# zyrlia1018/CMD-GEN

Measured on AMD Instinct MI355X. Metric: denoising steps/sec, higher is better.
Workload: dtype f32

## Files before the change

### cmdgen_amd/csrc/cmdgen_api.hip

```cpp
#include "cmdgen_dev.h"
#include "../../include/cmdgen_hip.h"

#include <cmath>
#include <cstdarg>
#include <cstdio>
#include <cstring>
#include <cstdlib>
#include <map>
#include <string>
#include <vector>

void cmdgen_launch_eval(const EvalLaunch& a, const float* xh_phar, const float* xh_pocket,
                        const float* t_arr, const float4* coef, ChainState* chain, float* eps_phar,
                        float* eps_pocket, hipStream_t s, hipEvent_t* ev);
void cmdgen_launch_nan_fix(const EvalLaunch& a, float* eps_phar, hipStream_t s);
void cmdgen_readout_allow_lds(size_t bytes);
void cmdgen_launch_edges(const EvalLaunch& a, const float* xh_phar, const float* xh_pocket, hipStream_t s);
void cmdgen_build_pocket_cache(const EvalLaunch& a, const float* xh_phar, const float* xh_pocket, const float* t01,
                               float* c, float* P0, float* Q0, float* dh, float* dP, float* dQ, hipStream_t s);
void cmdgen_launch_edge_msg_only(const EvalLaunch& a, int layer, hipStream_t s);
void cmdgen_launch_chain_init(const Layout& lay, const Dims& d, const ChainBuf& c, const float* px,
                              const float* poh, hipStream_t s);
void cmdgen_launch_step_count(const Layout& lay, const Dims& d, const ChainBuf& c, const Work& w,
                              const float* eps, hipStream_t s);
// ... 588 lines not shown
    const bool sp256 = h->dims.H == 256 && h->gemm_split;
    if (!sp256) { if (a.edge_mt == 128) a.edge_mt = 64; if (a.coord_mt == 128) a.coord_mt = 64; }
    if (h->dims.sin && h->dims.H == 512) { if (a.edge_mt > 32) a.edge_mt = 32; if (a.coord_mt > 32) a.coord_mt = 32; }
    a.edge_fullk = (sp256 && opt_of(h, "edge_fullk", 1) != 0) ? 1 : 0;
    a.e128_wgs = (int)opt_of(h, "e128_wgs_per_cu", 2);
    a.e128_fused = h->e128_fused;
    {
        const int he = (int)opt_of(h, "half_engine", 1);
        a.half_engine = he == 2 || (he == 1 && h->dims.cutoff2 >= 0.f) ? 1 : 0;
    }
    a.write_embed = opt_of(h, "write_embed", 1) != 0 ? 1 : 0;
    {
        int on = 0;
        if (sp256 && h->n_cus > 0 && h->have_layout) {
            const int ncu = h->n_cus, t64 = (h->lay.N + 63) / 64, t32 = (h->lay.N + 31) / 32;
            const float cost64 = (float)((t64 + ncu - 1) / ncu);
            const int full = t32 / (2 * ncu), rem = t32 - full * 2 * ncu;
            float cost32 = 1.12f * full + (rem == 0 ? 0.f : rem <= ncu ? 0.62f : 1.12f);
            if (a.half_engine) cost32 = 1.9f * full + (rem == 0 ? 0.f : rem <= ncu ? 1.22f : 1.9f);
            on = cost64 < cost32 && !(a.half_engine && h->node_mt == 16);
            if (a.half_engine && h->node_mt != 16) on = 32;
            if (on == 32 && t32 > ncu && t64 <= ncu) on = 8;
            else if (on == 32 && t64 > ncu) on = 2;
            if (opt_set(h, "node64")) { const int64_t v = opt_of(h, "node64", 0); on = v == 32 ? 32 : v == 8 ? 8 : v == 2 ? 2 : v != 0; }
        }
        a.node64 = on;
        a.dead_skip = (h->dims.joint || h->dims.S != 1) ? 0 : (int)opt_of(h, "dead_skip", 2);
        if (!on && !a.dead_skip) a.w.need_qc = nullptr;
        a.w.hop_levels = a.dead_skip >= 2 ? h->dims.L : 1;
        if (!a.dead_skip) a.w.ehop = nullptr;
    }
    a.split16 = (a.split && h->dims.H >= 128 && opt_of(h, "node16_split", 1) != 0) ? 1 : 0;
    a.node16w = opt_of(h, "node16w", 1) != 0 ? 1 : 0;
    {
        a.embed_mt = (int)opt_of(h, "embed_mt", (((double)h->lay.Nl / 16.0 <= 2.0 * h->n_cus && !h->dims.joint) ? 16 : a.node_mt));
        if (a.embed_mt != 16 && a.embed_mt != 32 && a.embed_mt != 64) a.embed_mt = a.node_mt;
    }
    if (a.split && a.node_mt == 64 && !opt_set(h, "node_mt")) a.node_mt = 32;
    return a;
}

static const char* const kOptionKeys[] = {
    "node_mt", "edge_mt", "coord_mt", "embed_mt", "edge_wgs_per_cu", "coord_wgs_per_cu", "e128_wgs_per_cu", "e128_fused", "half_engine", "edge_fullk", "node64", "node16_split", "node16w",
    "dead_skip", "write_embed", "graph_steps",
    "wgrad_split", "wgrad_tile", "wgrad_split_wgs128", "wgrad_split_wgs64", "wgrad_wgs", "dgrad_mt", "dgrad_tail", "wgrad_stream", "train_half", "wgrad_silu", "train_node16", "wgrad_k128"};

static void drop_graphs(cmdgen_handle* h) {
    hipSetDevice(h->device);
    if (h->own_stream) hipStreamSynchronize(h->own_stream);
    if (h->have_layout) hipStreamSynchronize(h->last_stream);
    drop_chain_graphs(h);
}
static void refresh_tune(cmdgen_handle* h) {
    TrainTune t;
    t.wgrad_split = (int)opt_of(h, "wgrad_split", t.wgrad_split); t.wgrad_tile = (int)opt_of(h, "wgrad_tile", t.wgrad_tile);
    t.wgrad_split_wgs128 = (int)opt_of(h, "wgrad_split_wgs128", t.wgrad_split_wgs128); t.wgrad_split_wgs64 = (int)opt_of(h, "wgrad_split_wgs64", t.wgrad_split_wgs64);
    t.wgrad_wgs = (int)opt_of(h, "wgrad_wgs", t.wgrad_wgs); t.dgrad_mt = (int)opt_of(h, "dgrad_mt", t.dgrad_mt); t.dgrad_tail = (int)opt_of(h, "dgrad_tail", t.dgrad_tail);
    t.wgrad_stream = (int)opt_of(h, "wgrad_stream", t.wgrad_stream); t.wgrad_k128 = (int)opt_of(h, "wgrad_k128", t.wgrad_k128);
    h->tune = t;
}

extern "C" int cmdgen_set_option(cmdgen_handle* h, const char* key, int64_t value, int32_t unset) {
    if (!h || !key) return fail(h, CMDGEN_EINVAL, "null argument");
    bool known = false;
    for (const char* k : kOptionKeys) known = known || strcmp(k, key) == 0;
    if (!known) return fail(h, CMDGEN_EINVAL, "unknown option '%s'", key);
    drop_graphs(h);
    if (unset) h->opts.erase(key); else h->opts[key] = value;
    refresh_tune(h);
    if (h->have_layout) pick_tiles(h);
    return CMDGEN_OK;
}

extern "C" int cmdgen_get_option(cmdgen_handle* h, const char* key, int64_t* value, int32_t* is_set) {
    if (!h || !key) return fail(h, CMDGEN_EINVAL, "null argument");
    bool known = false;
// ... 63 lines not shown
    TMP(w.ed0, float, need); TMP(w.totals, int, 4); TMP(w.counters, unsigned long long, 8); TMP(w.nan_flag, int, 4);
#undef TMP
    if (rc) { free_pool(pool); return rc; }
    w.erow = row_dev; w.ecol = col_dev;
    hipMemcpy(d_np, cnt.data(), B * sizeof(int), hipMemcpyHostToDevice);
    hipMemcpy(d_base, base.data(), B * sizeof(int), hipMemcpyHostToDevice);
    L.B = B; L.Nl = 0; L.Np = (int)N; L.N = (int)N; L.Nm = 0; L.max_n = max_n;
    L.num_phar = d_zero; L.num_pocket = d_np; L.phar_base = d_zero; L.pocket_base = d_base;
    EvalLaunch a{}; a.lay = L; a.w = w; a.d = d;
    cmdgen_launch_edges(a, x , x, s);
    hipError_t e = hipStreamSynchronize(s);
    int tot[2] = {0, 0};
    if (e == hipSuccess) e = hipMemcpy(tot, w.totals, sizeof tot, hipMemcpyDeviceToHost);
    free_pool(pool);
    if (e != hipSuccess) return fail(h, CMDGEN_EHIP, "radius graph failed: %s", hipGetErrorString(e));
    *n_edges = tot[0];
    return CMDGEN_OK;
}

extern "C" int cmdgen_get_edges(cmdgen_handle* h, int32_t* row, int32_t* col, int64_t cap, int64_t* n_edges, cmdgen_stream stream) {
    int rc = check_ready(h); if (rc) return rc;
    hipSetDevice(h->device);
    hipStream_t s = (hipStream_t)stream;
    HIPCHK(h, hipStreamSynchronize(s));
    int tot[2];
    HIPCHK(h, hipMemcpy(tot, h->work.totals, sizeof tot, hipMemcpyDeviceToHost));
    if (n_edges) *n_edges = tot[0];
    const int64_t n = tot[0] < cap ? tot[0] : cap;
    if (n > 0 && row) HIPCHK(h, hipMemcpy(row, h->work.erow, n * sizeof(int), hipMemcpyDeviceToHost));
    if (n > 0 && col) HIPCHK(h, hipMemcpy(col, h->work.ecol, n * sizeof(int), hipMemcpyDeviceToHost));
    return CMDGEN_OK;
}

extern "C" int cmdgen_debug_read(cmdgen_handle* h, const char* what, float* host, size_t n, cmdgen_stream stream) {
    int rc = check_ready(h); if (rc) return rc;
    hipSetDevice(h->device);
    HIPCHK(h, hipStreamSynchronize((hipStream_t)stream));
    const void* src = nullptr; size_t have = 0;
    const std::string k = what ? what : "";
    const Dims& d = h->dims;
    if (k == "h") { src = h->work.h; have = (size_t)h->lay.N * d.H; }
    else if (k == "agg") { src = h->work.agg; have = (size_t)h->lay.N * d.H; }
    else if (k == "P") { src = h->work.P; have = (size_t)h->lay.N * d.H; }
    else if (k == "Q") { src = h->work.Q; have = (size_t)h->lay.N * d.H; }
    else if (k == "x0") { src = h->work.X0; have = (size_t)h->lay.Nm * 4; }
    else if (k == "xl") { src = h->work.XL; have = (size_t)d.L * h->lay.Nm * 4; }
    else if (k == "acc") { src = h->work.ACC; have = (size_t)d.L * h->lay.Nm * 4; }
    else return fail(h, CMDGEN_EINVAL, "unknown debug buffer '%s'", k.c_str());
    if (n > have) n = have;
    HIPCHK(h, hipMemcpy(host, src, n * sizeof(float), hipMemcpyDeviceToHost));
    return CMDGEN_OK;
}

static inline float softplus_f(float x) { return x > 20.f ? x : log1pf(expf(x)); }
static inline float logsigmoid_f(float x) { return -softplus_f(-x); }
static inline float sigmoid_h(float x) { return 1.0f / (1.0f + expf(-x)); }

static void build_step_table(const std::vector<float>& gamma, int T, int K, std::vector<float>& coef) {
    coef.assign((size_t)(K + 1) * 4, 0.f);
    for (int i = 0; i < K; ++i) {
        const int s = K - 1 - i;
        const float s_arr = (float)s / (float)K, t_arr = (float)(s + 1) / (float)K;
        const float g_s = gamma[(size_t)lrintf(s_arr * (float)T)], g_t = gamma[(size_t)lrintf(t_arr * (float)T)];
        const float sigma2_ts = -expm1f(softplus_f(g_s) - softplus_f(g_t));
        const float alpha_ts = expf(0.5f * (logsigmoid_f(-g_t) - logsigmoid_f(-g_s)));
        const float sigma_ts = sqrtf(sigma2_ts);
        const float sigma_s = sqrtf(sigmoid_h(g_s)), sigma_t = sqrtf(sigmoid_h(g_t));
        coef[i * 4 + 0] = alpha_ts;
        coef[i * 4 + 1] = sigma2_ts / alpha_ts / sigma_t;
        coef[i * 4 + 2] = sigma_ts * sigma_s / sigma_t;
        coef[i * 4 + 3] = t_arr;
    }
    const float g0 = gamma[0];
    coef[K * 4 + 0] = sqrtf(sigmoid_h(g0));
    coef[K * 4 + 1] = sqrtf(sigmoid_h(-g0));
    coef[K * 4 + 2] = expf(0.5f * g0);
    coef[K * 4 + 3] = 0.f;
}

extern "C" int cmdgen_set_step_table(cmdgen_handle* h, int32_t K, const float* coef_host) {
// ... 588 lines not shown
    if (which == 1) {
        if (h256 && a.split && sampler && a.node64 && lw.W3.ws) return a.half_engine && lw.W3.wh ? 3 : 6;
        if (h256 && a.node_mt == 16 && a.split16 && a.node16w && sampler && lw.W3.ws16) return a.half_engine && lw.W3.wh16 ? 3 : 6;
        if ((a.split && a.node_mt >= 32) || (a.split16 && a.node_mt == 16)) return 6;
        return 1;
    }
    const int mt = which == 0 ? a.edge_mt : a.coord_mt;
    const WPack& W = which == 0 ? lw.W2 : lw.W7;
    if (mt == 128 && h256 && a.split && sampler && W.ws) return a.half_engine && W.wh ? 3 : 6;
    if (a.edge_fullk && sampler && a.split && h256 && mt == 32) return a.half_engine && W.wh ? 3 : 6;
    if (a.split && mt >= 32) return 6;
    return 1;
}

extern "C" int cmdgen_query(cmdgen_handle* h, const char* key, int64_t* value) {
    if (!h || !key || !value) return CMDGEN_EINVAL;
    if (!h->have_layout) return fail(h, CMDGEN_ESTATE, "no batch layout (cmdgen_set_layout)");
    const std::string k = key;
    const EvalLaunch a = make_launch(h);
    if (k == "node_mt") *value = a.node_mt;
    else if (k == "edge_mt") *value = a.edge_mt;
    else if (k == "e128_fused") *value = a.e128_fused;
    else if (k == "coord_mt") *value = a.coord_mt;
    else if (k == "edge_grid") *value = a.edge_grid;
    else if (k == "coord_grid") *value = a.coord_grid;
    else if (k == "gemm_split") *value = a.split;
    else if (k == "half_engine") *value = a.split ? a.half_engine : 0;
    else if (k == "msg_mfmas_per_product") *value = mfmas_per_product(a, 0);
    else if (k == "node_mfmas_per_product") *value = mfmas_per_product(a, 1);
    else if (k == "coord_mfmas_per_product") *value = mfmas_per_product(a, 2);
    else if (k == "node16_split") *value = a.split16;
    else if (k == "node64") *value = a.node64;
    else if (k == "node16w") *value = a.node16w;
    else if (k == "edge_fullk") *value = a.edge_fullk;
    else if (k == "dead_skip") *value = a.dead_skip;
    else if (k == "eval_gen") *value = h->eval_gen;
    else if (k == "train_half_ran") *value = h->train_fwd_half;
    else if (k == "train_range_event") *value = h->h_norm && !h->norm_pending ? (int64_t)h->h_norm[1] : 0;
    else if (k == "train_edges") *value = h->train_E;
    else if (k == "train_coord_edges") *value = h->train_Ec;
    else return fail(h, CMDGEN_EINVAL, "unknown query '%s'", key);
    return CMDGEN_OK;
}

extern "C" int cmdgen_time_evaluation(cmdgen_handle* h, const float* xh_phar, const float* xh_pocket, const float* t,
                                      float* eps_phar, int32_t graph_len, int32_t replays, float* mean_ms, cmdgen_stream stream) {
    int rc = check_ready(h); if (rc) return rc;
    if (!xh_phar || !xh_pocket || !t || !eps_phar || !mean_ms || graph_len < 1 || replays < 1) return fail(h, CMDGEN_EINVAL, "bad arguments");
    if (h->dims.joint) return fail(h, CMDGEN_ESTATE, "cmdgen_time_evaluation supports the conditional model only");
    hipStream_t caller = (hipStream_t)stream, s = caller;
    if (caller == nullptr) {
        rc = own_stream(h); if (rc) return rc;
        HIPCHK(h, hipDeviceSynchronize());
        s = h->own_stream;
    }
    rc = begin_work(h, s); if (rc) return rc;
    EvalLaunch a = make_launch(h);
    ++h->eval_gen;
    hipGraph_t g = nullptr; hipGraphExec_t ge = nullptr;
    hipEvent_t e0 = nullptr, e1 = nullptr;
    hipError_t err = hipStreamBeginCapture(s, hipStreamCaptureModeThreadLocal);
    if (err != hipSuccess) return fail(h, CMDGEN_EHIP, "hipStreamBeginCapture: %s", hipGetErrorString(err));
    for (int i = 0; i < graph_len; ++i) {
        cmdgen_launch_eval(a, xh_phar, xh_pocket, t, nullptr, nullptr, eps_phar, nullptr, s, nullptr);
        cmdgen_launch_nan_fix(a, eps_phar, s);
    }
// ... 92 lines not shown
```

### cmdgen_amd/csrc/cmdgen_dev.h

```cpp
#pragma once
#include <hip/hip_runtime.h>
#include <stdint.h>
#include <vector>
#include "cmdgen_split.h"

typedef float f32x16 __attribute__((ext_vector_type(16)));

#define CMDGEN_MAX_LAYERS 16
#define CMDGEN_MAX_SMALL 64


struct WPack {
    const float4* w32;
    const float4* w16;
    const void*   ws;
    const void*   ws16;
    const void*   wh;
    const void*   wh16;
    float         wh_scale;
    float         wh_inv;
    const float*  wh_dev;
};

struct LayerW {
// ... 161 lines not shown
    int slot;
};

struct TrainTune {
    int wgrad_split = -1;
    int wgrad_tile = 0;
    int wgrad_k128 = 131072;
    int wgrad_split_wgs128 = 384, wgrad_split_wgs64 = 512;
    int wgrad_wgs = 768;
    int dgrad_mt = 0;
    int dgrad_tail = 1;
    unsigned long long* dbg = nullptr;
    int wgrad_stream = 1;
};

struct EvalLaunch {
    Layout lay; Work w; Dims d; SmallW sw;
    const LayerW* layers;
    int edge_grid, coord_grid;
    int node_mt, edge_mt, coord_mt;
    int embed_mt = 16;
    std::vector<hipEvent_t>* prof_events;
    mutable hipEvent_t pe_start = nullptr, pe_stop = nullptr;
    int ablate;
    int stop_block = -1, stop_stage = 0;
    const TrainSave* save = nullptr;
    PocketCache pcache{};
    int skip_count = 0;
    int split = 0;
    int split16 = 0;
    int n_cus = 256;
    int edge_fullk = 0;
    int node16w = 1;
    int node64 = 0;
    int dead_skip = 0;
    mutable int unit = -1;
    mutable int skip_pc = 0;
    mutable int frag_launches = 0;
    mutable int live_thr = 0;
    int save_half = 0;
    int save_half16 = 0;
    int save_split = 0;
    int write_embed = 1;
    int e128_wgs = 2;
    int e128_fused = 3;
    int half_engine = 1;
};
inline int unit_of(const EvalLaunch& a, int l) { return a.unit >= 0 ? a.unit : l; }
inline int unit_has_next(const EvalLaunch& a, int l) { return unit_of(a, l) + 1 < a.d.L * a.d.S ? 1 : 0; }
inline int node_flags(const EvalLaunch& a, int l) { return unit_has_next(a, l) | (a.live_thr << 1) | (a.skip_pc << 30); }


__device__ __forceinline__ float silu_f(float v) {
    return v * __builtin_amdgcn_rcpf(1.0f + __builtin_amdgcn_exp2f(-1.4426950408889634f * v));
}
__device__ __forceinline__ float sigmoid_f(float v) {
    return __builtin_amdgcn_rcpf(1.0f + __builtin_amdgcn_exp2f(-1.4426950408889634f * v));
}
__device__ __forceinline__ float dist2(const float4& a, const float4& b) {
    const float dx = a.x - b.x, dy = a.y - b.y, dz = a.z - b.z;
    return __fmaf_rn(dz, dz, __fmaf_rn(dy, dy, dx * dx));
}

typedef float f32x4v __attribute__((ext_vector_type(4)));

template <int MT> struct TileAcc;
// ... 249 lines not shown
```

### cmdgen_amd/csrc/cmdgen_node16w_body.h

```cpp
#ifndef NW_RD_HALF
#define NW_RD_HALF 8
#endif
constexpr int NW_H = 256, NW_MT = 16, NW_LD = NW_H + 4 , NW_RD = NW_NPL == 2 ? NW_RD_HALF : 4;
constexpr int NPL = NW_NPL;
constexpr unsigned KBS = 64u * NPL;
#if NW_NPL == 3
typedef sbf16x8 wfrag;
#define NW_MFMA(A, B, C) __builtin_amdgcn_mfma_f32_16x16x32_bf16(A, B, C, 0, 0, 0)
#else
typedef sf16x8 wfrag;
#define NW_MFMA(A, B, C) __builtin_amdgcn_mfma_f32_16x16x32_f16(A, B, C, 0, 0, 0)
#endif
__device__ __forceinline__ const void* nw_pack(const WPack& W) { return NPL == 3 ? W.ws16 : W.wh16; }
__device__ __forceinline__ float nw_scale(const WPack& W) { return NPL == 3 ? 1.0f : W.wh_scale; }
__device__ __forceinline__ float nw_inv(const WPack& W) { return NPL == 3 ? 1.0f : W.wh_inv; }

__device__ __forceinline__ void nw_barrier() { asm volatile("s_waitcnt lgkmcnt(0)\n\ts_barrier" ::: "memory"); }

struct NwFrag { const wfrag* p; unsigned ns; };
__device__ __forceinline__ NwFrag nw_frag(const void* Ws16, int kb32_total, int kb0, int nt0) {
    const int lane = threadIdx.x & 63;
    NwFrag f;
    f.p = reinterpret_cast<const wfrag*>(Ws16) + ((size_t)nt0 * kb32_total + kb0) * KBS + lane;
    f.ns = (unsigned)kb32_total * KBS;
    return f;
}
struct NwRing { wfrag b[NW_RD][2][NPL]; };
__device__ __forceinline__ void nw_load_set(const wfrag* q, unsigned ns, wfrag (&dst)[2][NPL]) {
#pragma unroll
    for (int n = 0; n < 2; ++n)
#pragma unroll
        for (int s = 0; s < NPL; ++s) dst[n][s] = q[n * ns + s * 64];
}
__device__ __forceinline__ void nw_prefetch(const NwFrag& f, NwRing& c) {
#pragma unroll
    for (int i = 0; i < NW_RD - 1; ++i) nw_load_set(f.p + i * KBS, f.ns, c.b[i]);
}

#if NW_NPL == 3
__device__ __forceinline__ void nw_split8(const float4& lo, const float4& hi, wfrag (&p)[NPL]) { split8(lo, hi, p[0], p[1], p[2]); }
#else
__device__ __forceinline__ void nw_split8(const float4& lo, const float4& hi, wfrag (&p)[NPL]) {
    {
        uint32_t a[4], b[4];
        split2_pair(lo.x, lo.y, a[0], b[0]); split2_pair(lo.z, lo.w, a[1], b[1]);
        split2_pair(hi.x, hi.y, a[2], b[2]); split2_pair(hi.z, hi.w, a[3], b[3]);
        typedef uint32_t u4 __attribute__((ext_vector_type(4)));
        const u4 va = {a[0], a[1], a[2], a[3]}, vb = {b[0], b[1], b[2], b[3]};
        p[0] = __builtin_bit_cast(wfrag, va); p[1] = __builtin_bit_cast(wfrag, vb);
    }
}
#endif

template <int KB32>
__device__ __forceinline__ void nw_gemm(const float* ldsA, const NwFrag cur, const NwFrag next, sf32x4 (&acc)[2], NwRing& ring) {
    static_assert(KB32 % NW_RD == 0 && (NW_RD == 4 || NW_RD == 8), "K must be a multiple of the ring's k-range");
    const int lane = threadIdx.x & 63;
    const float* ap = ldsA + (lane & 15) * NW_LD + (lane >> 4) * 4;
    float4 raw[2][2];
    wfrag a[2][NPL];
#define NW_LOADA(SET, PTR) { raw[SET][0] = *reinterpret_cast<const float4*>(PTR); raw[SET][1] = *reinterpret_cast<const float4*>((PTR) + 16); }
#define NW_SPLIT(DST, SET) nw_split8(raw[SET][0], raw[SET][1], a[DST]);
#define NW_MF(AS, AI, BS, BI) _Pragma("unroll") for (int n = 0; n < 2; ++n) acc[n] = NW_MFMA(a[AS][AI], ring.b[BS][n][BI], acc[n]);
#if NW_NPL == 3
#define NW_MFMAS(AS, BS) NW_MF(AS, 2, BS, 0) NW_MF(AS, 1, BS, 1) NW_MF(AS, 0, BS, 2) NW_MF(AS, 1, BS, 0) NW_MF(AS, 0, BS, 1) NW_MF(AS, 0, BS, 0)
#define NW_INTERLEAVE()                                                                                                     \
    _Pragma("unroll") for (int i = 0; i < 12; ++i) {                                                                        \
        __builtin_amdgcn_sched_group_barrier(0x008, 1, 0);                                                                  \
        __builtin_amdgcn_sched_group_barrier(0x002, 4, 0); }
// ... 33 lines not shown
}

template <class F>
__device__ __forceinline__ void nw_foreach(const sf32x4 (&acc)[2], int wave, F f) {
    const int lane = threadIdx.x & 63;
#pragma unroll
    for (int n = 0; n < 2; ++n)
#pragma unroll
        for (int r = 0; r < 4; ++r) f(4 * (lane >> 4) + r, wave * 32 + n * 16 + (lane & 15), n, acc[n][r]);
}
struct NwCol { float v[2]; };
__device__ __forceinline__ NwCol nw_col(const float* __restrict__ vec, int wave) {
    const int lane = threadIdx.x & 63;
    NwCol c;
#pragma unroll
    for (int n = 0; n < 2; ++n) c.v[n] = vec[wave * 32 + n * 16 + (lane & 15)];
    return c;
}
__device__ __forceinline__ void nw_zero(sf32x4 (&acc)[2]) {
#pragma unroll
    for (int n = 0; n < 2; ++n)
#pragma unroll
        for (int r = 0; r < 4; ++r) acc[n][r] = 0.0f;
}
__device__ __forceinline__ void nw_store(const sf32x4 (&acc)[2], int wave, float* __restrict__ out, int row0, int nvalid, const NwCol* bias, float inv) {
    nw_foreach(acc, wave, [&](int row, int col, int n, float v) {
        if (row < nvalid) out[(size_t)(row0 + row) * NW_H + col] = __fmaf_rn(v, inv, bias ? bias->v[n] : 0.f);
    });
}
__device__ __forceinline__ float nw_silu_scaled(float a, float c1, float sc) {
    const float u = __builtin_amdgcn_exp2f(a * c1);
    return a * __builtin_amdgcn_rcpf(__fmaf_rn(u, sc, sc));
}
template <bool SAVE>
__global__ __launch_bounds__(512) void k_node16w(Layout lay, Work w, Dims d, LayerW lw, LayerW lw_next, int layer, int has_next_arg, TrainSave sv) {
    __shared__ __attribute__((aligned(16))) float buf0[NW_MT * NW_LD];
    __shared__ __attribute__((aligned(16))) float buf1[NW_MT * NW_LD];
    const int has_next = has_next_arg & 1;
    const bool skip_pc = ((has_next_arg >> 30) & 1) != 0;
    const int tid = threadIdx.x, wave = tid >> 6;
    const int row0 = (int)blockIdx.x * NW_MT, nvalid = min(NW_MT, lay.N - row0);
    const bool want_pc = row0 < lay.Nm;
    constexpr int KB = NW_H / 32;
    const NwFrag f3a = nw_frag(nw_pack(lw.W3), 2 * KB, 0, 2 * wave), f3b = nw_frag(nw_pack(lw.W3), 2 * KB, KB, 2 * wave);
    const NwFrag f4 = nw_frag(nw_pack(lw.W4), KB, 0, 2 * wave);
    const NwFrag fcp = nw_frag(nw_pack(lw.Wpq_c), KB, 0, 2 * wave), fcq = nw_frag(nw_pack(lw.Wpq_c), KB, 0, NW_H / 16 + 2 * wave);
    const NwFrag fnp = nw_frag(nw_pack(lw_next.Wpq_e), KB, 0, 2 * wave), fnq = nw_frag(nw_pack(lw_next.Wpq_e), KB, 0, NW_H / 16 + 2 * wave);
    NwRing ring;
    nw_prefetch(f3a, ring);
    NwCol b3v = nw_col(lw.b3, wave);
    const NwCol b4v = nw_col(lw.b4, wave), b6v = nw_col(lw.b6, wave), b1nv = nw_col(lw_next.b1, wave);
    float sc3 = nw_scale(lw.W3), inv3 = nw_inv(lw.W3), inv4 = nw_inv(lw.W4), invc = nw_inv(lw.Wpq_c), invn = nw_inv(lw_next.Wpq_e);
    if constexpr (SAVE) { sc3 = lw.W3.wh_dev[0]; inv3 = lw.W3.wh_dev[1]; inv4 = lw.W4.wh_dev[1]; invc = lw.Wpq_c.wh_dev[1]; invn = lw_next.Wpq_e.wh_dev[1]; }
    const float c13 = -1.4426950408889634f * inv3;
    b3v.v[0] *= sc3; b3v.v[1] *= sc3;
    if (layer >= 1 && tid < NW_MT) {
        const int n = row0 + tid;
        if (tid < nvalid && n < lay.Nm) {
            const float4 p = (layer == 1) ? w.X0[n] : w.XL[(size_t)(layer - 1) * lay.Nm + n];
            const float4 a = w.ACC[(size_t)(layer - 1) * lay.Nm + n];
            const float dv = agg_div(w, d, n);
            w.XL[(size_t)layer * lay.Nm + n] = make_float4(p.x + a.x / dv, p.y + a.y / dv, p.z + a.z / dv, 0.f);
        }
    }
    {
        float4 hv[2], av[2];
#pragma unroll
        for (int j = 0; j < 2; ++j) {
            const int idx = tid + 512 * j, r = idx >> 6, c4 = idx & 63;
            hv[j] = make_float4(0.f, 0.f, 0.f, 0.f); av[j] = hv[j];
            if (r < nvalid) {
                hv[j] = reinterpret_cast<const float4*>(w.h + (size_t)(row0 + r) * NW_H)[c4];
                av[j] = reinterpret_cast<const float4*>(w.agg + (size_t)(row0 + r) * NW_H)[c4];
            }
        }
#pragma unroll
        for (int j = 0; j < 2; ++j) {
            const int idx = tid + 512 * j, r = idx >> 6, c4 = idx & 63;
            if (r < nvalid) reinterpret_cast<float4*>(w.agg + (size_t)(row0 + r) * NW_H)[c4] = make_float4(0.f, 0.f, 0.f, 0.f);
            float4 v = av[j];
            const float dv = r < nvalid ? agg_div(w, d, row0 + r) : 1.0f;
            v.x /= dv; v.y /= dv; v.z /= dv; v.w /= dv;
            if (SAVE && r < nvalid) reinterpret_cast<float4*>(sv.aggn + ((size_t)sv.slot * lay.N + row0 + r) * NW_H)[c4] = v;
            *reinterpret_cast<float4*>(buf0 + r * NW_LD + 4 * c4) = hv[j];
            *reinterpret_cast<float4*>(buf1 + r * NW_LD + 4 * c4) = v;
        }
    }
#if CMDGEN_STAMPS == 7
    unsigned long long nst_[8] = {0, 0, 0, 0, 0, 0, 0, 0}, nst_t = __builtin_amdgcn_s_memtime();
    const unsigned long long nst_begin = nst_t;
#define NSTAMP(i) do { const unsigned long long n_ = __builtin_amdgcn_s_memtime(); nst_[i] += n_ - nst_t; nst_t = n_; } while (0)
#else
#define NSTAMP(i) do {} while (0)
#endif
    nw_barrier();
    NSTAMP(0);
    sf32x4 acc[2];
    nw_zero(acc);
    nw_gemm<KB>(buf0, f3a, f3b, acc, ring);
    nw_gemm<KB>(buf1, f3b, f4, acc, ring);
    NSTAMP(1);
    nw_barrier();
    nw_foreach(acc, wave, [&](int row, int col, int n, float v) {
        const float t = nw_silu_scaled(v + b3v.v[n], c13, sc3);
        buf1[row * NW_LD + col] = t;
        if (SAVE && row < nvalid) {
            const size_t o = ((size_t)sv.slot * lay.N + row0 + row) * NW_H + col;
            sv.pre3[o] = (v + b3v.v[n]) * inv3; sv.nact[o] = t;
        }
    });
    nw_barrier();
    NSTAMP(2);
    nw_zero(acc);
    const NwFrag fc = skip_pc ? fnp : want_pc ? fcp : fcq;
    nw_gemm<KB>(buf1, f4, fc, acc, ring);
    if constexpr (NPL == 2) {
        const int row = tid >> 5, c8 = (tid & 31) * 8;
        const float m = fmaxf(absmax4(*reinterpret_cast<const float4*>(buf1 + row * NW_LD + c8)), absmax4(*reinterpret_cast<const float4*>(buf1 + row * NW_LD + c8 + 4)));
        const unsigned long long big = __ballot(m >= HALF_LOW_TAU);
        const int r0 = 2 * wave;
        if ((tid & 63) == 0) half_low_count(w.counters, (r0 < nvalid && (unsigned)big == 0u ? 1u : 0u) + (r0 + 1 < nvalid && (big >> 32) == 0ull ? 1u : 0u));
    }
    NSTAMP(3);
    nw_barrier();
    nw_foreach(acc, wave, [&](int row, int col, int n, float v) {
        float hn = 0.f;
        if (row < nvalid) {
            hn = buf0[row * NW_LD + col] + __fmaf_rn(v, inv4, b4v.v[n]);
            w.h[(size_t)(row0 + row) * NW_H + col] = hn;
            if (SAVE) sv.h[((size_t)(sv.slot + 1) * lay.N + row0 + row) * NW_H + col] = hn;
        }
        buf1[row * NW_LD + col] = hn;
    });
    nw_barrier();
    NSTAMP(4);
    if (want_pc && !skip_pc) {
        nw_zero(acc);
        nw_gemm<KB>(buf1, fcp, fcq, acc, ring);
        nw_store(acc, wave, w.Pc, row0, nvalid, &b6v, invc);
    }
    if (!skip_pc) {
        nw_zero(acc);
        nw_gemm<KB>(buf1, fcq, has_next ? fnp : fcq, acc, ring);
        nw_store(acc, wave, w.Qc, row0, nvalid, nullptr, invc);
    }
    NSTAMP(5);
    if (has_next) {
        nw_zero(acc);
        nw_gemm<KB>(buf1, fnp, fnq, acc, ring);
        nw_store(acc, wave, w.P, row0, nvalid, &b1nv, invn);
        nw_zero(acc);
        nw_gemm<KB>(buf1, fnq, fnq, acc, ring);
        nw_store(acc, wave, w.Q, row0, nvalid, nullptr, invn);
    }
    NSTAMP(6);
#if CMDGEN_STAMPS == 7
    if ((tid & 63) == 0 && wave < 4) {
        for (int i = 0; i < 7; ++i) atomicAdd(&w.dbg[wave * 8 + i], nst_[i]);
        atomicAdd(&w.dbg[32 + wave], __builtin_amdgcn_s_memtime() - nst_begin);
        atomicAdd(&w.dbg[40], 1ull);
    }
#endif
#undef NSTAMP
}
```

### cmdgen_amd/csrc/cmdgen_train.hip

```cpp
#include "cmdgen_host.h"
#include <functional>

void cmdgen_launch_edges(const EvalLaunch& a, const float* xh_phar, const float* xh_pocket, hipStream_t s);
void cmdgen_launch_eval(const EvalLaunch& a, const float* xh_phar, const float* xh_pocket, const float* t_arr, const float4* coef,
                        ChainState* chain, float* eps_phar, float* eps_pocket, hipStream_t s, hipEvent_t* ev);
void cmdgen_launch_nan_fix(const EvalLaunch& a, float* eps_phar, hipStream_t s);
void cmdgen_launch_save_positions(const EvalLaunch& a, float4* X, hipStream_t s);
struct RepackFrag { int src_off, ld, out, in, row_split, col_shift; float* dst32; float* dst16; };
struct RepackMisc { int src_off, ld, rows, cols; float* dst; };
void tr_repack(const float* theta, const void* frag_tab, int n_frag, int max_frag4, const void* misc_tab, int n_misc, int max_misc,
               hipStream_t s);
void cmdgen_sgemm(bool ta, bool tb, int M, int N, int K, const float* A, int lda, const float* B, int ldb, float* C,
                  int ldc, const float* bias, float alpha, bool accumulate, int split_k, hipStream_t s,
                  int epi = 0, float* aux = nullptr, int ldaux = 0, bool bf16 = false);
struct WgradBatch {
    const float* dy[8]; const float* x[8]; float* dw[8]; float* db[8];
    int M[8], N[8], lddy[8], ldx[8], ldw[8];
    int n;
    int xs[8] = {0, 0, 0, 0, 0, 0, 0, 0};
};
void cmdgen_wgrad_group(const WgradBatch& g, int K, bool bf16, hipStream_t s, bool split3 = false, bool force3 = false);
struct RepackSplitT { int src_off, ld; void* dst; int transpose; };
void tr_repack_split_t(const float* theta, const void* tab, int n, hipStream_t s);
struct RepackHalf { int src_off, ld; void* dst; float* sc; int transpose; };
// ... 351 lines not shown
                   bool bias, bool accumulate, hipStream_t s, float* act = nullptr) {
    cmdgen_sgemm(false, true, M, r.out, in, x, ldx, theta + r.w + col0, r.in, y, ldy, (bias && r.has_bias) ? theta + r.b : nullptr,
                 1.0f, accumulate, 1, s, act ? 1 : 0, act, ldy, use_bf16(in));
}
static void linear_dgrad(const float* theta, const PRef& r, int col0, int in, int M, const float* dy, int lddy, float* dx,
                         int lddx, bool accumulate, hipStream_t s, const float* pre = nullptr) {
    cmdgen_sgemm(false, false, M, in, r.out, dy, lddy, theta + r.w + col0, r.in, dx, lddx, nullptr, 1.0f, accumulate, 1, s,
                 pre ? 2 : 0, const_cast<float*>(pre), lddx, use_bf16(r.out));
}
static void linear_wgrad(float* grad, const PRef& r, int col0, int in, int M, const float* dy, int lddy, const float* x,
                         int ldx, hipStream_t s) {
    cmdgen_sgemm(true, false, r.out, in, M, dy, lddy, x, ldx, grad + r.w + col0, r.in, nullptr, 1.0f, true, 0, s, 0, nullptr, 0,
                 g_bf16 && r.out >= 64 && in >= 64);
}

extern "C" int cmdgen_param_count(cmdgen_handle* h, int64_t* n) {
    if (!h || !n) return CMDGEN_EINVAL;
    ParamTable t; build_table(h->dims, t);
    *n = (int64_t)t.total;
    return CMDGEN_OK;
}

extern "C" int cmdgen_param_offset(cmdgen_handle* h, const char* name, int64_t* offset, int64_t* count) {
    if (!h || !name) return CMDGEN_EINVAL;
    ParamTable t; build_table(h->dims, t);
    const std::string k = name;
    for (const PRef* r : t.order) {
        if (k == r->name + ".weight") { if (offset) *offset = (int64_t)r->w; if (count) *count = (int64_t)r->out * r->in; return CMDGEN_OK; }
        if (r->has_bias && k == r->name + ".bias") { if (offset) *offset = (int64_t)r->b; if (count) *count = r->out; return CMDGEN_OK; }
    }
    return fail(h, CMDGEN_EINVAL, "no trainable tensor '%s'", name);
}

extern "C" int cmdgen_train_forward(cmdgen_handle* h, const float* theta, const float* xh_phar, const float* xh_pocket,
                                    const float* t_arr, float* eps_phar, float* eps_pocket, cmdgen_stream stream) {
    if (!h) return CMDGEN_EINVAL;
    if (!h->have_layout) return fail(h, CMDGEN_ESTATE, "no batch layout (cmdgen_set_layout)");
    if (!theta || !xh_phar || !xh_pocket || !t_arr || !eps_phar) return fail(h, CMDGEN_EINVAL, "null device pointer");
    if (h->dims.joint && !eps_pocket) return fail(h, CMDGEN_EINVAL, "the joint model's loss needs eps_pocket");
    hipSetDevice(h->device);
    int rc = ensure_state(h); if (rc) return rc;
    TrainState* t = h->train;
    hipStream_t s = (hipStream_t)stream;
    h->last_stream = s;
    const Dims& d = h->dims;
    const int N = h->lay.N, Nl = h->lay.Nl, Np = h->lay.Np, H = d.H, L = d.L, P = d.P, R = d.R, J = d.J;
    const int ldp = 3 + P, ldq = 3 + R, ld1 = 2 * H + 2;
    EvalLaunch a = make_launch(h);
    ++h->eval_gen;
    a.dead_skip = 0; a.w.need_qc = nullptr; a.w.ehop = nullptr; a.w.hop_levels = 1;
    cmdgen_launch_edges(a, xh_phar, xh_pocket, s);
    if (!t->h_tot) {
        HIPCHK(h, hipHostMalloc((void**)&t->h_tot, 4 * sizeof(int), hipHostMallocDefault));
        HIPCHK(h, hipEventCreateWithFlags(&t->tot_ev, hipEventDisableTiming));
    }
    HIPCHK(h, hipMemcpyAsync(t->h_tot, h->work.totals, 2 * sizeof(int), hipMemcpyDeviceToHost, s));
    HIPCHK(h, hipEventRecord(t->tot_ev, s));
    const bool fwd_half = h->gemm_split && H == 256 && a.half_engine && a.edge_fullk && t->n_half > 0 && opt_of(h, "train_half", 1) != 0;
    if (fwd_half && opt_of(h, "train_node16", 1) != 0) a.node_mt = 16;
    const bool node_half = fwd_half && a.node_mt == 16 && t->n_half16 > 0 && opt_of(h, "train_half", 1) != 2;
    const bool frag_partial = fwd_half && node_half;
    tr_repack(theta, t->frag_tab, frag_partial ? 1 : t->n_frag, t->max_frag4, t->misc_tab, t->n_misc, t->max_misc, s);
    if (h->gemm_split || t->bf16) tr_repack_split_t(theta, t->split_tab, t->n_split, s);
    t->split_packs_valid = (h->gemm_split || t->bf16) && t->n_split > 0;
    if (fwd_half) tr_repack_half(theta, t->half_tab, t->n_half_fwd, t->n_half_fwd, s);
    if (node_half) tr_repack_half16(theta, t->half16_tab, t->n_half16, t->max_half16, s);
// ... 583 lines not shown
```

### cmdgen_amd/csrc/kernels_node16w.hip

```cpp
#include "cmdgen_dev.h"
#include "cmdgen_split.h"
#include <hip/hip_ext.h>

#define NW_NPL 2
namespace nw_half {
#include "cmdgen_node16w_body.h"
}
#undef NW_NPL
#undef NW_MFMA
#define NW_NPL 3
namespace nw_bf3 {
#include "cmdgen_node16w_body.h"
}
#undef NW_NPL
#undef NW_MFMA

bool cmdgen_launch_node16w(const EvalLaunch& a, int l, hipStream_t s) {
    const LayerW& lw = a.layers[unit_of(a, l)];
    const LayerW& ln = a.layers[unit_has_next(a, l) ? unit_of(a, l) + 1 : unit_of(a, l)];
    const int nt = (a.lay.N + 15) / 16;
    if (a.save) {
        if (a.d.H != 256 || a.node_mt != 16 || !a.save_half16 || !lw.W3.wh16 || !lw.W3.wh_dev) return false;
        TrainSave sv = *a.save; sv.slot = unit_of(a, l);
        hipLaunchKernelGGL(nw_half::k_node16w<true>, dim3(nt), dim3(512), 0, s, a.lay, a.w, a.d, lw, ln, l, node_flags(a, l), sv);
        return true;
    }
    if (a.d.H != 256 || a.node_mt != 16 || !a.split16 || !a.node16w || !lw.W3.ws16) return false;
    if (a.half_engine && lw.W3.wh16) {
        if (a.pe_start) hipExtLaunchKernelGGL(nw_half::k_node16w<false>, dim3(nt), dim3(512), 0, s, a.pe_start, a.pe_stop, 0, a.lay, a.w, a.d, lw, ln, l, node_flags(a, l), TrainSave{});
        else hipLaunchKernelGGL(nw_half::k_node16w<false>, dim3(nt), dim3(512), 0, s, a.lay, a.w, a.d, lw, ln, l, node_flags(a, l), TrainSave{});
    } else {
        if (a.pe_start) hipExtLaunchKernelGGL(nw_bf3::k_node16w<false>, dim3(nt), dim3(512), 0, s, a.pe_start, a.pe_stop, 0, a.lay, a.w, a.d, lw, ln, l, node_flags(a, l), TrainSave{});
        else hipLaunchKernelGGL(nw_bf3::k_node16w<false>, dim3(nt), dim3(512), 0, s, a.lay, a.w, a.d, lw, ln, l, node_flags(a, l), TrainSave{});
    }
    return true;
}
```

Before: 182,700.

## Pipeline node16w kernel: issue activation loads before weight prefetch, triple-buffer LDS

Adds a PIPE variant of the node16w kernel, enabled by default. It issues the h/agg and coordinate loads first, then does the weight-ring prefetch with scheduling barriers that keep it in order. A third LDS buffer holds the SiLU output so two block-wide barriers can be dropped. The aim is to overlap global-load latency with weight prefetch and cut synchronisation stalls. In exchange it uses extra shared memory, which may lower occupancy, and it adds debug buffers and timing stamps.

```diff
diff --git a/cmdgen_amd/csrc/cmdgen_api.hip b/cmdgen_amd/csrc/cmdgen_api.hip
--- a/cmdgen_amd/csrc/cmdgen_api.hip
+++ b/cmdgen_amd/csrc/cmdgen_api.hip
@@ -644,6 +644,7 @@
     }
     a.split16 = (a.split && h->dims.H >= 128 && opt_of(h, "node16_split", 1) != 0) ? 1 : 0;
     a.node16w = opt_of(h, "node16w", 1) != 0 ? 1 : 0;
+    a.node16w_pipe = opt_of(h, "node16w_pipe", 1) != 0 ? 1 : 0;
     {
         a.embed_mt = (int)opt_of(h, "embed_mt", (((double)h->lay.Nl / 16.0 <= 2.0 * h->n_cus && !h->dims.joint) ? 16 : a.node_mt));
         if (a.embed_mt != 16 && a.embed_mt != 32 && a.embed_mt != 64) a.embed_mt = a.node_mt;
@@ -653,7 +654,7 @@
 }
 
 static const char* const kOptionKeys[] = {
-    "node_mt", "edge_mt", "coord_mt", "embed_mt", "edge_wgs_per_cu", "coord_wgs_per_cu", "e128_wgs_per_cu", "e128_fused", "half_engine", "edge_fullk", "node64", "node16_split", "node16w",
+    "node_mt", "edge_mt", "coord_mt", "embed_mt", "edge_wgs_per_cu", "coord_wgs_per_cu", "e128_wgs_per_cu", "e128_fused", "half_engine", "edge_fullk", "node64", "node16_split", "node16w", "node16w_pipe",
     "dead_skip", "write_embed", "graph_steps",
     "wgrad_split", "wgrad_tile", "wgrad_split_wgs128", "wgrad_split_wgs64", "wgrad_wgs", "dgrad_mt", "dgrad_tail", "wgrad_stream", "train_half", "wgrad_silu", "train_node16", "wgrad_k128"};
 
@@ -783,6 +784,7 @@
     return CMDGEN_OK;
 }
 
+bool cmdgen_train_debug_buffer(const cmdgen_handle* h, const std::string& what, const void** src, size_t* count);
 extern "C" int cmdgen_debug_read(cmdgen_handle* h, const char* what, float* host, size_t n, cmdgen_stream stream) {
     int rc = check_ready(h); if (rc) return rc;
     hipSetDevice(h->device);
@@ -797,6 +799,7 @@
     else if (k == "x0") { src = h->work.X0; have = (size_t)h->lay.Nm * 4; }
     else if (k == "xl") { src = h->work.XL; have = (size_t)d.L * h->lay.Nm * 4; }
     else if (k == "acc") { src = h->work.ACC; have = (size_t)d.L * h->lay.Nm * 4; }
+    else if (cmdgen_train_debug_buffer(h, k, &src, &have)) {}
     else return fail(h, CMDGEN_EINVAL, "unknown debug buffer '%s'", k.c_str());
     if (n > have) n = have;
     HIPCHK(h, hipMemcpy(host, src, n * sizeof(float), hipMemcpyDeviceToHost));
@@ -1451,6 +1454,7 @@
     else if (k == "node16_split") *value = a.split16;
     else if (k == "node64") *value = a.node64;
     else if (k == "node16w") *value = a.node16w;
+    else if (k == "node16w_pipe") *value = a.node16w_pipe;
     else if (k == "edge_fullk") *value = a.edge_fullk;
     else if (k == "dead_skip") *value = a.dead_skip;
     else if (k == "eval_gen") *value = h->eval_gen;
diff --git a/cmdgen_amd/csrc/cmdgen_dev.h b/cmdgen_amd/csrc/cmdgen_dev.h
--- a/cmdgen_amd/csrc/cmdgen_dev.h
+++ b/cmdgen_amd/csrc/cmdgen_dev.h
@@ -217,6 +217,7 @@
     int n_cus = 256;
     int edge_fullk = 0;
     int node16w = 1;
+    int node16w_pipe = 1;
     int node64 = 0;
     int dead_skip = 0;
     mutable int unit = -1;
diff --git a/cmdgen_amd/csrc/cmdgen_node16w_body.h b/cmdgen_amd/csrc/cmdgen_node16w_body.h
--- a/cmdgen_amd/csrc/cmdgen_node16w_body.h
+++ b/cmdgen_amd/csrc/cmdgen_node16w_body.h
@@ -35,6 +35,12 @@
 __device__ __forceinline__ void nw_prefetch(const NwFrag& f, NwRing& c) {
 #pragma unroll
     for (int i = 0; i < NW_RD - 1; ++i) nw_load_set(f.p + i * KBS, f.ns, c.b[i]);
+}
+
+__device__ __forceinline__ void nw_prefetch_in_order(const NwFrag& f, NwRing& c) {
+#pragma unroll
+    for (int i = 0; i < NW_RD - 1; ++i) { __builtin_amdgcn_sched_barrier(0); nw_load_set(f.p + i * KBS, f.ns, c.b[i]); }
+    __builtin_amdgcn_sched_barrier(0);
 }
 
 #if NW_NPL == 3
@@ -134,13 +140,18 @@
     const float u = __builtin_amdgcn_exp2f(a * c1);
     return a * __builtin_amdgcn_rcpf(__fmaf_rn(u, sc, sc));
 }
-template <bool SAVE>
+template <bool SAVE, int PIPE>
 __global__ __launch_bounds__(512) void k_node16w(Layout lay, Work w, Dims d, LayerW lw, LayerW lw_next, int layer, int has_next_arg, TrainSave sv) {
     __shared__ __attribute__((aligned(16))) float buf0[NW_MT * NW_LD];
     __shared__ __attribute__((aligned(16))) float buf1[NW_MT * NW_LD];
+    __shared__ __attribute__((aligned(16))) float buf2[PIPE ? NW_MT * NW_LD : 4];
+    float* const bufT = PIPE ? buf2 : buf1;
     const int has_next = has_next_arg & 1;
     const bool skip_pc = ((has_next_arg >> 30) & 1) != 0;
     const int tid = threadIdx.x, wave = tid >> 6;
+#if CMDGEN_STAMPS == 7
+    const unsigned long long nst_entry = __builtin_amdgcn_s_memtime();
+#endif
     const int row0 = (int)blockIdx.x * NW_MT, nvalid = min(NW_MT, lay.N - row0);
     const bool want_pc = row0 < lay.Nm;
     constexpr int KB = NW_H / 32;
@@ -149,14 +160,24 @@
     const NwFrag fcp = nw_frag(nw_pack(lw.Wpq_c), KB, 0, 2 * wave), fcq = nw_frag(nw_pack(lw.Wpq_c), KB, 0, NW_H / 16 + 2 * wave);
     const NwFrag fnp = nw_frag(nw_pack(lw_next.Wpq_e), KB, 0, 2 * wave), fnq = nw_frag(nw_pack(lw_next.Wpq_e), KB, 0, NW_H / 16 + 2 * wave);
     NwRing ring;
-    nw_prefetch(f3a, ring);
+    if constexpr (!PIPE) nw_prefetch(f3a, ring);
     NwCol b3v = nw_col(lw.b3, wave);
     const NwCol b4v = nw_col(lw.b4, wave), b6v = nw_col(lw.b6, wave), b1nv = nw_col(lw_next.b1, wave);
     float sc3 = nw_scale(lw.W3), inv3 = nw_inv(lw.W3), inv4 = nw_inv(lw.W4), invc = nw_inv(lw.Wpq_c), invn = nw_inv(lw_next.Wpq_e);
     if constexpr (SAVE) { sc3 = lw.W3.wh_dev[0]; inv3 = lw.W3.wh_dev[1]; inv4 = lw.W4.wh_dev[1]; invc = lw.Wpq_c.wh_dev[1]; invn = lw_next.Wpq_e.wh_dev[1]; }
     const float c13 = -1.4426950408889634f * inv3;
     b3v.v[0] *= sc3; b3v.v[1] *= sc3;
-    if (layer >= 1 && tid < NW_MT) {
+    const bool xl = layer >= 1 && tid < NW_MT && tid < nvalid && row0 + tid < lay.Nm;
+    float4 xl_p = make_float4(0.f, 0.f, 0.f, 0.f), xl_a = xl_p;
+    float xl_dv = 1.0f;
+    if constexpr (PIPE) {
+        if (xl) {
+            const int n = row0 + tid;
+            xl_p = (layer == 1) ? w.X0[n] : w.XL[(size_t)(layer - 1) * lay.Nm + n];
+            xl_a = w.ACC[(size_t)(layer - 1) * lay.Nm + n];
+            xl_dv = agg_div(w, d, n);
+        }
+    } else if (layer >= 1 && tid < NW_MT) {
         const int n = row0 + tid;
         if (tid < nvalid && n < lay.Nm) {
             const float4 p = (layer == 1) ? w.X0[n] : w.XL[(size_t)(layer - 1) * lay.Nm + n];
@@ -165,7 +186,33 @@
             w.XL[(size_t)layer * lay.Nm + n] = make_float4(p.x + a.x / dv, p.y + a.y / dv, p.z + a.z / dv, 0.f);
         }
     }
-    {
+    if constexpr (PIPE) {
+        float4 hv[2], av[2];
+        float dv[2];
+#pragma unroll
+        for (int j = 0; j < 2; ++j) {
+            const int idx = tid + 512 * j, r = idx >> 6, c4 = idx & 63, rr = r < nvalid ? r : 0;
+            hv[j] = reinterpret_cast<const float4*>(w.h + (size_t)(row0 + rr) * NW_H)[c4];
+            av[j] = reinterpret_cast<const float4*>(w.agg + (size_t)(row0 + rr) * NW_H)[c4];
+        }
+#pragma unroll
+        for (int j = 0; j < 2; ++j) dv[j] = agg_div(w, d, row0 + (tid >> 6) + 8 * j < lay.N ? row0 + (tid >> 6) + 8 * j : row0);
+        nw_prefetch_in_order(f3a, ring);
+        if (xl) w.XL[(size_t)layer * lay.Nm + row0 + tid] = make_float4(xl_p.x + xl_a.x / xl_dv, xl_p.y + xl_a.y / xl_dv, xl_p.z + xl_a.z / xl_dv, 0.f);
+#pragma unroll
+        for (int j = 0; j < 2; ++j) {
+            const int idx = tid + 512 * j, r = idx >> 6, c4 = idx & 63;
+            const bool ok = r < nvalid;
+            if (ok) reinterpret_cast<float4*>(w.agg + (size_t)(row0 + r) * NW_H)[c4] = make_float4(0.f, 0.f, 0.f, 0.f);
+            float4 v = av[j], hj = hv[j];
+            if (!ok) { v.x = 0.f; v.y = 0.f; v.z = 0.f; v.w = 0.f; hj = v; }
+            const float dvj = ok ? dv[j] : 1.0f;
+            v.x /= dvj; v.y /= dvj; v.z /= dvj; v.w /= dvj;
+            if (SAVE && ok) reinterpret_cast<float4*>(sv.aggn + ((size_t)sv.slot * lay.N + row0 + r) * NW_H)[c4] = v;
+            *reinterpret_cast<float4*>(buf0 + r * NW_LD + 4 * c4) = hj;
+            *reinterpret_cast<float4*>(buf1 + r * NW_LD + 4 * c4) = v;
+        }
+    } else {
         float4 hv[2], av[2];
 #pragma unroll
         for (int j = 0; j < 2; ++j) {
@@ -202,10 +249,10 @@
     nw_gemm<KB>(buf0, f3a, f3b, acc, ring);
     nw_gemm<KB>(buf1, f3b, f4, acc, ring);
     NSTAMP(1);
-    nw_barrier();
+    if constexpr (!PIPE) nw_barrier();
     nw_foreach(acc, wave, [&](int row, int col, int n, float v) {
         const float t = nw_silu_scaled(v + b3v.v[n], c13, sc3);
-        buf1[row * NW_LD + col] = t;
+        bufT[row * NW_LD + col] = t;
         if (SAVE && row < nvalid) {
             const size_t o = ((size_t)sv.slot * lay.N + row0 + row) * NW_H + col;
             sv.pre3[o] = (v + b3v.v[n]) * inv3; sv.nact[o] = t;
@@ -215,16 +262,16 @@
     NSTAMP(2);
     nw_zero(acc);
     const NwFrag fc = skip_pc ? fnp : want_pc ? fcp : fcq;
-    nw_gemm<KB>(buf1, f4, fc, acc, ring);
+    nw_gemm<KB>(bufT, f4, fc, acc, ring);
     if constexpr (NPL == 2) {
         const int row = tid >> 5, c8 = (tid & 31) * 8;
-        const float m = fmaxf(absmax4(*reinterpret_cast<const float4*>(buf1 + row * NW_LD + c8)), absmax4(*reinterpret_cast<const float4*>(buf1 + row * NW_LD + c8 + 4)));
+        const float m = fmaxf(absmax4(*reinterpret_cast<const float4*>(bufT + row * NW_LD + c8)), absmax4(*reinterpret_cast<const float4*>(bufT + row * NW_LD + c8 + 4)));
         const unsigned long long big = __ballot(m >= HALF_LOW_TAU);
         const int r0 = 2 * wave;
         if ((tid & 63) == 0) half_low_count(w.counters, (r0 < nvalid && (unsigned)big == 0u ? 1u : 0u) + (r0 + 1 < nvalid && (big >> 32) == 0ull ? 1u : 0u));
     }
     NSTAMP(3);
-    nw_barrier();
+    if constexpr (!PIPE) nw_barrier();
     nw_foreach(acc, wave, [&](int row, int col, int n, float v) {
         float hn = 0.f;
         if (row < nvalid) {
@@ -261,6 +308,7 @@
         for (int i = 0; i < 7; ++i) atomicAdd(&w.dbg[wave * 8 + i], nst_[i]);
         atomicAdd(&w.dbg[32 + wave], __builtin_amdgcn_s_memtime() - nst_begin);
         atomicAdd(&w.dbg[40], 1ull);
+        atomicAdd(&w.dbg[44 + wave], nst_begin - nst_entry);
     }
 #endif
 #undef NSTAMP
diff --git a/cmdgen_amd/csrc/cmdgen_train.hip b/cmdgen_amd/csrc/cmdgen_train.hip
--- a/cmdgen_amd/csrc/cmdgen_train.hip
+++ b/cmdgen_amd/csrc/cmdgen_train.hip
@@ -407,6 +407,18 @@
     return fail(h, CMDGEN_EINVAL, "no trainable tensor '%s'", name);
 }
 
+bool cmdgen_train_debug_buffer(const cmdgen_handle* h, const std::string& what, const void** src, size_t* count) {
+    const TrainState* t = h->train;
+    if (!t || !t->have_forward) return false;
+    const size_t U = (size_t)h->dims.L * h->dims.S, NH = (size_t)h->lay.N * h->dims.H;
+    if (what == "save_aggn") { *src = t->aggn; *count = U * NH; }
+    else if (what == "save_pre3") { *src = t->pre3; *count = U * NH; }
+    else if (what == "save_nact") { *src = t->nact; *count = U * NH; }
+    else if (what == "save_h") { *src = t->h; *count = (U + 1) * NH; }
+    else return false;
+    return true;
+}
+
 extern "C" int cmdgen_train_forward(cmdgen_handle* h, const float* theta, const float* xh_phar, const float* xh_pocket,
                                     const float* t_arr, float* eps_phar, float* eps_pocket, cmdgen_stream stream) {
     if (!h) return CMDGEN_EINVAL;
diff --git a/cmdgen_amd/csrc/kernels_node16w.hip b/cmdgen_amd/csrc/kernels_node16w.hip
--- a/cmdgen_amd/csrc/kernels_node16w.hip
+++ b/cmdgen_amd/csrc/kernels_node16w.hip
@@ -22,16 +22,18 @@
     if (a.save) {
         if (a.d.H != 256 || a.node_mt != 16 || !a.save_half16 || !lw.W3.wh16 || !lw.W3.wh_dev) return false;
         TrainSave sv = *a.save; sv.slot = unit_of(a, l);
-        hipLaunchKernelGGL(nw_half::k_node16w<true>, dim3(nt), dim3(512), 0, s, a.lay, a.w, a.d, lw, ln, l, node_flags(a, l), sv);
+        if (a.node16w_pipe) hipLaunchKernelGGL((nw_half::k_node16w<true, 1>), dim3(nt), dim3(512), 0, s, a.lay, a.w, a.d, lw, ln, l, node_flags(a, l), sv);
+        else hipLaunchKernelGGL((nw_half::k_node16w<true, 0>), dim3(nt), dim3(512), 0, s, a.lay, a.w, a.d, lw, ln, l, node_flags(a, l), sv);
         return true;
     }
     if (a.d.H != 256 || a.node_mt != 16 || !a.split16 || !a.node16w || !lw.W3.ws16) return false;
-    if (a.half_engine && lw.W3.wh16) {
-        if (a.pe_start) hipExtLaunchKernelGGL(nw_half::k_node16w<false>, dim3(nt), dim3(512), 0, s, a.pe_start, a.pe_stop, 0, a.lay, a.w, a.d, lw, ln, l, node_flags(a, l), TrainSave{});
-        else hipLaunchKernelGGL(nw_half::k_node16w<false>, dim3(nt), dim3(512), 0, s, a.lay, a.w, a.d, lw, ln, l, node_flags(a, l), TrainSave{});
-    } else {
-        if (a.pe_start) hipExtLaunchKernelGGL(nw_bf3::k_node16w<false>, dim3(nt), dim3(512), 0, s, a.pe_start, a.pe_stop, 0, a.lay, a.w, a.d, lw, ln, l, node_flags(a, l), TrainSave{});
-        else hipLaunchKernelGGL(nw_bf3::k_node16w<false>, dim3(nt), dim3(512), 0, s, a.lay, a.w, a.d, lw, ln, l, node_flags(a, l), TrainSave{});
+#define NW_LAUNCH(NS, PIPE)                                                                                                                                          \
+    {                                                                                                                                                                \
+        if (a.pe_start) hipExtLaunchKernelGGL((NS::k_node16w<false, PIPE>), dim3(nt), dim3(512), 0, s, a.pe_start, a.pe_stop, 0, a.lay, a.w, a.d, lw, ln, l, node_flags(a, l), TrainSave{}); \
+        else hipLaunchKernelGGL((NS::k_node16w<false, PIPE>), dim3(nt), dim3(512), 0, s, a.lay, a.w, a.d, lw, ln, l, node_flags(a, l), TrainSave{});                    \
     }
+    if (a.half_engine && lw.W3.wh16) { if (a.node16w_pipe) NW_LAUNCH(nw_half, 1) else NW_LAUNCH(nw_half, 0) }
+    else { if (a.node16w_pipe) NW_LAUNCH(nw_bf3, 1) else NW_LAUNCH(nw_bf3, 0) }
+#undef NW_LAUNCH
     return true;
 }
```

Result: no change. 183,700, median of 6 (+0.5%).
